# matteobutano/optimal_crowds

Hardware: NVIDIA B200
Metric: hjb_gcell_updates_per_s (higher is better)
Workload: dtype f64

## Files before the change

### include/optimal_crowds.h

```cpp
#ifndef OPTIMAL_CROWDS_H
#define OPTIMAL_CROWDS_H

#include <stdint.h>

#ifdef __cplusplus
extern "C" {
#endif

#define OC_ABI_VERSION 2

typedef enum {
    OC_OK = 0,
    OC_ERR_CUDA = -1,
    OC_ERR_ARG = -2,
    OC_ERR_NOMEM = -3,
    OC_ERR_SAMPLER_RANGE = -4,
    OC_ERR_STEP_TOO_SMALL = -5,
    OC_ERR_NCCL = -6
} oc_status;

typedef struct oc_ctx oc_ctx;

int oc_abi_version(void);
const char *oc_last_error(void);
long long oc_launch_count(int reset);

int oc_ctx_create(int device, int Ny, int Nx, double dx, double dy, double room_length, double room_height,
                  const double *X, const double *Y, oc_ctx **out);
void oc_ctx_destroy(oc_ctx *ctx);
int oc_ctx_set_int(oc_ctx *ctx, const char *key, int value);

int oc_upload(oc_ctx *ctx, const void *host, void *d_dst, long long bytes, void *stream);

long long oc_place_box(const double *box, const double *X, int Nx, const double *Y, int Ny, double *place_ped, double r_in,
                       uint32_t *mt_key, int *mt_pos, double *xs, double *ys, int loc_N);

int oc_rng_step_draw(uint32_t *mt_key, int *mt_pos, int *has_gauss, double *cached_gauss, int N, int n_active, int *perm,
                     double *noise);
int oc_rng_step_draw_ckpt(uint32_t *mt_key, int *mt_pos, int *has_gauss, double *cached_gauss, int N, int n_active,
                          int *perm, double *noise, int n_ckpt, uint32_t *ckpt_key, int *ckpt_pos, int *ckpt_has,
                          double *ckpt_cached);

int oc_rasterise(oc_ctx *ctx, const double *walls, int n_walls, const double *holes, int n_holes,
                 const double *cyls, int n_cyls, const double *targets, int n_targets, int remap,
                 double wall_value, double target_value, double *d_V, void *stream);

typedef struct {
    double sigma, mu, g;
    double rtol, atol;
    double lim;
    int fused;
    int profile;
    const double *forced_h;
    int n_forced_h;
    int chunk_rows;
} oc_hjb_params;

typedef struct {
    int nfev;
    int n_accepted;
    int n_rejected;
    int status;
    int n_out;
    int launches;
    double h0;
    double gpu_ms;
    int cls_launches[3];
    int pad_;
    double cls_ms[3];
    double cls_bytes[3];
} oc_hjb_stats;

int oc_hjb_solve(oc_ctx *ctx, const double *d_V, const double *d_m, const oc_hjb_params *prm, double T,
                 const double *t_eval, int nt, double *d_phi, double *d_vx, double *d_vy, oc_hjb_stats *stats,
                 double *trace_h, double *trace_err, int trace_cap, int *trace_n, void *stream);

int oc_hjb_plan_chunk_rows(oc_ctx *ctx, int copies);
int oc_hjb_solve_batch(oc_ctx *ctx, int n_rooms, const double *const *d_V, const double *const *d_m,
                       const oc_hjb_params *prm, double T, const double *t_eval, int nt, double *const *d_phi,
                       double *const *d_vx, double *const *d_vy, oc_hjb_stats *stats, void *stream);

typedef struct {
    int n_virtual;
    int own0, own1;
    int phi_extra_hi;
} oc_band_cfg;
int oc_dist_unique_id(void *out128);
int oc_dist_init(oc_ctx *ctx, const void *id128, int rank, int nranks);
int oc_dist_finalize(oc_ctx *ctx);
int oc_dist_p2p_export(oc_ctx *ctx, int band_rows, void *handle_out64);
int oc_dist_p2p_import(oc_ctx *ctx, const void *handles, int n);
int oc_dist_p2p_enabled(oc_ctx *ctx);
int oc_dist_p2p_disable(oc_ctx *ctx);
int oc_hjb_solve_band(oc_ctx *ctx, const oc_band_cfg *cfg, const double *d_V, const double *d_m,
                      const oc_hjb_params *prm, double T, const double *t_eval, int nt, double *d_phi, double *d_vx,
                      double *d_vy, oc_hjb_stats *stats, double *trace_h, double *trace_err, int trace_cap,
                      int *trace_n, void *stream);
int oc_rasterise_band(oc_ctx *ctx, const double *walls, int n_walls, const double *holes, int n_holes,
                      const double *cyls, int n_cyls, const double *targets, int n_targets, int remap,
                      double wall_value, double target_value, int row0, int rows, double *d_V, void *stream);

int oc_hjb_rhs(oc_ctx *ctx, const double *d_phi, const double *d_V, const double *d_m, const oc_hjb_params *prm,
               double *d_out, void *stream);
int oc_hjb_vels(oc_ctx *ctx, const double *d_phi, const oc_hjb_params *prm, double *d_vx, double *d_vy,
                void *stream);

typedef struct {
    double dt, dt2, half_noise, relaxation, v_max, cutoff;
    double a_min, tau_a, b_min, b_max, eta, eta_walls;
    double cos_fov, one_minus_cos_fov;
    double dx, dy, room_length, room_height;
    int Ny, Nx;
    int own0, own1;
    int key_mod, key_rem;
} oc_gcfm_params;

typedef struct {
    const double *d_V;
    const uint8_t *d_wall_tiles;
    double v_min;
    const double *d_vx, *d_vy;
    int nt_opt;
    int n_slices;
    const double *d_phi;
    int n_phi;
    int pad_;
    double mu, lim;
    const double *doors;
// ... 54 lines not shown
```

### optimal_crowds_b200/_lib.py

```python
from __future__ import annotations

import ctypes as C
import os

import numpy as np

_HERE = os.path.dirname(os.path.abspath(__file__))
LIB_PATH = os.environ.get("OC_B200_LIB") or os.path.join(_HERE, "liboc_b200.so")

dp = C.POINTER(C.c_double)
ip = C.POINTER(C.c_int)
u8p = C.POINTER(C.c_uint8)


class OcError(RuntimeError):
    def __init__(self, code, msg):
        super().__init__(f"liboc_b200 error {code}: {msg}")
        self.code = code


OC_ERR_SAMPLER_RANGE = -4
OC_ERR_STEP_TOO_SMALL = -5


class HjbParams(C.Structure):
    _fields_ = [("sigma", C.c_double), ("mu", C.c_double), ("g", C.c_double), ("rtol", C.c_double),
                ("atol", C.c_double), ("lim", C.c_double), ("fused", C.c_int), ("profile", C.c_int),
                ("forced_h", dp), ("n_forced_h", C.c_int), ("chunk_rows", C.c_int)]

    def force_steps(self, h):
        if h is None:
            self._keep = None
            self.forced_h, self.n_forced_h = None, 0
        else:
            self._keep = np.ascontiguousarray(h, dtype=np.float64)
            self.forced_h, self.n_forced_h = self._keep.ctypes.data_as(dp), len(self._keep)
        return self


class HjbStats(C.Structure):
    _fields_ = [("nfev", C.c_int), ("n_accepted", C.c_int), ("n_rejected", C.c_int), ("status", C.c_int),
                ("n_out", C.c_int), ("launches", C.c_int), ("h0", C.c_double), ("gpu_ms", C.c_double),
                ("cls_launches", C.c_int * 3), ("pad_", C.c_int), ("cls_ms", C.c_double * 3),
                ("cls_bytes", C.c_double * 3)]

    def asdict(self):
        d = {f: getattr(self, f) for f, _ in self._fields_ if not f.startswith(("cls_", "pad_"))}
        for f in ("cls_launches", "cls_ms", "cls_bytes"):
            d[f] = list(getattr(self, f))
        return d


class BandCfg(C.Structure):
    _fields_ = [("n_virtual", C.c_int), ("own0", C.c_int), ("own1", C.c_int), ("phi_extra_hi", C.c_int)]


class GcfmParams(C.Structure):
    _fields_ = [(n, C.c_double) for n in
                ("dt", "dt2", "half_noise", "relaxation", "v_max", "cutoff", "a_min", "tau_a", "b_min", "b_max",
                 "eta", "eta_walls", "cos_fov", "one_minus_cos_fov", "dx", "dy", "room_length", "room_height")] + \
               [("Ny", C.c_int), ("Nx", C.c_int), ("own0", C.c_int), ("own1", C.c_int), ("key_mod", C.c_int),
                ("key_rem", C.c_int)]


class Key(C.Structure):
    _fields_ = [("d_V", C.c_void_p), ("d_wall_tiles", C.c_void_p), ("v_min", C.c_double), ("d_vx", C.c_void_p),
                ("d_vy", C.c_void_p), ("nt_opt", C.c_int), ("n_slices", C.c_int), ("d_phi", C.c_void_p),
                ("n_phi", C.c_int), ("pad_", C.c_int), ("mu", C.c_double), ("lim", C.c_double), ("doors", dp),
                ("n_doors", C.c_int), ("phi_row0", C.c_int), ("phi_rows", C.c_int)]


_lib = None

EXPORTS = ["oc_abi_version", "oc_last_error", "oc_launch_count", "oc_ctx_create", "oc_ctx_destroy", "oc_ctx_set_int", "oc_rasterise",
           "oc_hjb_solve", "oc_hjb_rhs", "oc_hjb_vels", "oc_wall_tiles_bytes", "oc_wall_tiles", "oc_gcfm_step",
           "oc_wall_force", "oc_pair_force", "oc_density", "oc_gcfm_last_ms", "oc_dist_unique_id", "oc_dist_init",
           "oc_dist_finalize", "oc_dist_p2p_export", "oc_dist_p2p_import", "oc_dist_p2p_enabled", "oc_dist_p2p_disable", "oc_hjb_solve_band", "oc_rasterise_band", "oc_upload", "oc_hjb_solve_batch", "oc_gcfm_step_launch",
           "oc_gcfm_step_finish", "oc_gcfm_last_pairs", "oc_gcfm_last_redos", "oc_state_pack", "oc_fp64_peak", "oc_place_box", "oc_hjb_plan_chunk_rows", "oc_rng_step_draw", "oc_rng_step_draw_ckpt", "oc_gcfm_step_multi_launch", "oc_gcfm_step_multi_finish", "oc_gcfm_run"]


def load():
    global _lib
    if _lib is not None:
        return _lib
    if not os.path.exists(LIB_PATH):
        raise ImportError(f"{LIB_PATH} not found: build it with `python -m optimal_crowds_b200.build` "
                          "(the CUDA library is the only implementation; there is no CPU fallback)")
    lib = C.CDLL(LIB_PATH)
    lib.oc_last_error.restype = C.c_char_p
    lib.oc_launch_count.restype = C.c_longlong
    lib.oc_wall_tiles_bytes.restype = C.c_longlong
    lib.oc_gcfm_last_ms.restype = C.c_double
    lib.oc_gcfm_last_ms.argtypes = [C.c_void_p]
    lib.oc_gcfm_last_pairs.restype = C.c_longlong
    lib.oc_gcfm_last_pairs.argtypes = [C.c_void_p]
    lib.oc_gcfm_last_redos.argtypes = [C.c_void_p]
    lib.oc_state_pack.argtypes = [C.c_void_p, C.c_int] + [C.c_void_p] * 6
    lib.oc_fp64_peak.argtypes = [C.c_void_p, dp]
    lib.oc_hjb_plan_chunk_rows.argtypes = [C.c_void_p, C.c_int]
    vpp_ = C.POINTER(C.c_void_p)
    lib.oc_gcfm_step_multi_launch.argtypes = [C.c_int, vpp_, vpp_, ip] + [vpp_] * 9 + [ip, vpp_, ip, ip, dp, ip, ip,
                                                                                     C.c_int, C.c_void_p]
    lib.oc_gcfm_step_multi_finish.argtypes = [C.c_int, vpp_, vpp_, ip, ip]
    lib.oc_gcfm_run.argtypes = [C.c_void_p, C.POINTER(GcfmParams), C.c_int] + [C.c_void_p] * 8 + [C.c_void_p, C.c_int,
                                C.POINTER(C.c_uint32), ip, ip, dp, C.c_int, C.c_int, C.c_int, vpp_, ip, ip, ip, ip, dp,
                                C.POINTER(C.c_longlong), C.c_void_p]
    lib.oc_rng_step_draw.argtypes = [C.POINTER(C.c_uint32), ip, ip, dp, C.c_int, C.c_int, ip, dp]
    lib.oc_rng_step_draw_ckpt.argtypes = [C.POINTER(C.c_uint32), ip, ip, dp, C.c_int, C.c_int, ip, dp, C.c_int,
                                          C.POINTER(C.c_uint32), ip, ip, dp]
    lib.oc_place_box.restype = C.c_longlong
    lib.oc_place_box.argtypes = [dp, dp, C.c_int, dp, C.c_int, dp, C.c_double, C.POINTER(C.c_uint32), ip, dp, dp, C.c_int]
    lib.oc_wall_tiles_bytes.argtypes = [C.c_void_p]
    lib.oc_ctx_set_int.argtypes = [C.c_void_p, C.c_char_p, C.c_int]
    lib.oc_ctx_destroy.restype = None
    lib.oc_ctx_destroy.argtypes = [C.c_void_p]
    lib.oc_ctx_create.argtypes = [C.c_int, C.c_int, C.c_int, C.c_double, C.c_double, C.c_double, C.c_double, dp, dp,
                                  C.POINTER(C.c_void_p)]
    lib.oc_rasterise.argtypes = [C.c_void_p, dp, C.c_int, dp, C.c_int, dp, C.c_int, dp, C.c_int, C.c_int, C.c_double,
                                 C.c_double, C.c_void_p, C.c_void_p]
    lib.oc_hjb_solve.argtypes = [C.c_void_p, C.c_void_p, C.c_void_p, C.POINTER(HjbParams), C.c_double, dp, C.c_int,
                                 C.c_void_p, C.c_void_p, C.c_void_p, C.POINTER(HjbStats), dp, dp, C.c_int, ip,
                                 C.c_void_p]
    lib.oc_hjb_solve_band.argtypes = [C.c_void_p, C.POINTER(BandCfg), C.c_void_p, C.c_void_p, C.POINTER(HjbParams),
                                      C.c_double, dp, C.c_int, C.c_void_p, C.c_void_p, C.c_void_p, C.POINTER(HjbStats),
                                      dp, dp, C.c_int, ip, C.c_void_p]
    lib.oc_rasterise_band.argtypes = [C.c_void_p, dp, C.c_int, dp, C.c_int, dp, C.c_int, dp, C.c_int, C.c_int,
                                      C.c_double, C.c_double, C.c_int, C.c_int, C.c_void_p, C.c_void_p]
    vpp = C.POINTER(C.c_void_p)
    lib.oc_hjb_solve_batch.argtypes = [C.c_void_p, C.c_int, vpp, vpp, C.POINTER(HjbParams), C.c_double, dp, C.c_int,
                                       vpp, vpp, vpp, C.POINTER(HjbStats), C.c_void_p]
    lib.oc_upload.argtypes = [C.c_void_p, C.c_void_p, C.c_void_p, C.c_longlong, C.c_void_p]
    lib.oc_dist_unique_id.argtypes = [C.c_void_p]
    lib.oc_dist_init.argtypes = [C.c_void_p, C.c_void_p, C.c_int, C.c_int]
    lib.oc_dist_finalize.argtypes = [C.c_void_p]
    lib.oc_dist_p2p_export.argtypes = [C.c_void_p, C.c_int, C.c_void_p]
    lib.oc_dist_p2p_import.argtypes = [C.c_void_p, C.c_void_p, C.c_int]
    lib.oc_dist_p2p_enabled.argtypes = [C.c_void_p]
    lib.oc_dist_p2p_disable.argtypes = [C.c_void_p]
    lib.oc_hjb_rhs.argtypes = [C.c_void_p, C.c_void_p, C.c_void_p, C.c_void_p, C.POINTER(HjbParams), C.c_void_p,
                               C.c_void_p]
    lib.oc_hjb_vels.argtypes = [C.c_void_p, C.c_void_p, C.POINTER(HjbParams), C.c_void_p, C.c_void_p, C.c_void_p]
    lib.oc_wall_tiles.argtypes = [C.c_void_p, C.c_void_p, C.c_void_p, dp, C.c_void_p]
    lib.oc_gcfm_step.argtypes = [C.c_void_p, C.POINTER(GcfmParams), C.c_int] + [C.c_void_p] * 8 + \
                                [C.POINTER(Key), C.c_int, ip, dp, C.c_int, C.c_int, ip, ip, C.c_void_p]
    lib.oc_gcfm_step_launch.argtypes = [C.c_void_p, C.POINTER(GcfmParams), C.c_int] + [C.c_void_p] * 8 + \
                                       [C.POINTER(Key), C.c_int, ip, dp, C.c_int, C.c_int, C.c_void_p]
    lib.oc_gcfm_step_finish.argtypes = [C.c_void_p, ip, ip]
    lib.oc_wall_force.argtypes = [C.c_void_p, C.POINTER(GcfmParams), C.c_void_p, C.c_int] + [C.c_void_p] * 8 + \
                                 [C.c_void_p]
    lib.oc_pair_force.argtypes = [C.c_void_p, C.POINTER(GcfmParams), C.c_int] + [C.c_void_p] * 6 + [C.c_void_p]
    lib.oc_density.argtypes = [C.c_void_p, C.c_int, C.c_void_p, C.c_void_p, C.c_void_p, C.c_double, C.c_double,
                               C.c_void_p, C.c_void_p, C.c_void_p]
    _lib = lib
    return lib


def check(rc, allow=()):
    if rc != 0 and rc not in allow:
        raise OcError(rc, load().oc_last_error().decode())
    return rc


def _hp(a):
    return None if a is None else a.ctypes.data_as(dp)


def _dev(t):
    if t is None:
        return None
    assert t.is_cuda and t.is_contiguous(), "expected a contiguous CUDA tensor"
    return C.c_void_p(t.data_ptr())


def _stream():
    import torch
# ... 100 lines not shown
        t_eval = np.linspace(T, 0, nt)
        if n_virtual and n_virtual > 1 or own is None:
            rows, prow, own0, own1 = self.Ny, self.Ny, 0, self.Ny
            vshape = (max(nt - 1, 0), self.Ny - 2, self.Nx - 2)
        else:
            own0, own1 = own
            rows = own1 - own0
            prow = rows + 2 + int(phi_extra_hi)
            vshape = (max(nt - 1, 0), rows, self.Nx - 2)
        phi = out_phi if out_phi is not None else (self.empty(nt, prow, self.Nx) if want_phi else None)
        vx = vy = None
        if want_vel:
            import torch
            vx = torch.zeros(vshape, dtype=torch.float64, device=self.torch_device)
            vy = torch.zeros(vshape, dtype=torch.float64, device=self.torch_device)
        cfg = BandCfg(int(n_virtual or 0), int(own0), int(own1), int(phi_extra_hi))
        st = HjbStats()
        cap = 1 << 16 if trace else 0
        th = np.empty(max(cap, 1)); te = np.empty(max(cap, 1))
        ntr = C.c_int()
        rc = load().oc_hjb_solve_band(self.h, C.byref(cfg), _dev(V), _dev(m), C.byref(prm), float(T), _hp(t_eval),
                                      int(nt), _dev(phi), _dev(vx), _dev(vy), C.byref(st), _hp(th) if trace else None,
                                      _hp(te) if trace else None, cap, C.byref(ntr), _stream())
        check(rc, allow=(OC_ERR_STEP_TOO_SMALL,))
        res = {"stats": st.asdict(), "phi": phi, "vx": vx, "vy": vy, "rc": rc}
        if trace:
            k = min(ntr.value, cap)
            res["trace_h"], res["trace_err"] = th[:k].copy(), te[:k].copy()
        return res

    def hjb_solve(self, V, m, prm: HjbParams, T, nt, want_phi=False, want_vel=True, trace=False, out_vx=None,
                  out_vy=None, out_phi=None):
        t_eval = np.linspace(T, 0, nt)
        n = self.Ny * self.Nx
        phi = out_phi if out_phi is not None else (self.empty(nt, self.Ny, self.Nx) if want_phi else None)
        vx = vy = None
        if want_vel:
            vx = out_vx if out_vx is not None else self.empty(max(nt - 1, 0), self.Ny - 2, self.Nx - 2)
            vy = out_vy if out_vy is not None else self.empty(max(nt - 1, 0), self.Ny - 2, self.Nx - 2)
        st = HjbStats()
        cap = 1 << 16 if trace else 0
        th = np.empty(max(cap, 1)); te = np.empty(max(cap, 1))
        ntr = C.c_int()
        rc = load().oc_hjb_solve(self.h, _dev(V), _dev(m), C.byref(prm), float(T), _hp(t_eval), int(nt), _dev(phi),
                                 _dev(vx), _dev(vy), C.byref(st), _hp(th) if trace else None,
                                 _hp(te) if trace else None, cap, C.byref(ntr), _stream())
        check(rc, allow=(OC_ERR_STEP_TOO_SMALL,))
        res = {"stats": st.asdict(), "phi": phi, "vx": vx, "vy": vy, "rc": rc}
        if trace:
            k = min(ntr.value, cap)
            res["trace_h"], res["trace_err"] = th[:k].copy(), te[:k].copy()
        return res

    def hjb_solve_batch(self, Vs, ms, prm: HjbParams, T, nt, out_phi=None, out_vx=None, out_vy=None, want_vel=False):
        B = len(Vs)
        t_eval = np.linspace(T, 0, nt)
        if out_phi is None and not (want_vel or out_vx is not None):
            out_phi = [self.empty(nt, self.Ny, self.Nx) for _ in range(B)]
        if want_vel and out_vx is None:
            out_vx = [self.empty(max(nt - 1, 0), self.Ny - 2, self.Nx - 2) for _ in range(B)]
            out_vy = [self.empty(max(nt - 1, 0), self.Ny - 2, self.Nx - 2) for _ in range(B)]

        def ptrs(ts):
            if ts is None:
                return None
            arr = (C.c_void_p * B)()
            for q, t in enumerate(ts):
                if t is not None:
                    assert t.is_cuda and t.is_contiguous()
                    arr[q] = t.data_ptr()
            return arr
        st = (HjbStats * B)()
        rc = load().oc_hjb_solve_batch(self.h, B, ptrs(Vs), ptrs(ms), C.byref(prm), float(T), _hp(t_eval), int(nt),
                                       ptrs(out_phi), ptrs(out_vx), ptrs(out_vy), st, _stream())
        check(rc, allow=(OC_ERR_STEP_TOO_SMALL,))
        return [{"stats": st[q].asdict(), "phi": out_phi[q] if out_phi is not None else None,
                 "vx": out_vx[q] if out_vx is not None else None, "vy": out_vy[q] if out_vx is not None else None,
                 "rc": rc if st[q].status == -1 else 0} for q in range(B)]

    def plan_chunk_rows(self, copies=1):
        rc = int(load().oc_hjb_plan_chunk_rows(self.h, int(copies)))
        check(min(rc, 0))
        return rc

    def hjb_rhs(self, phi, V, m, prm: HjbParams):
        out = self.empty(self.Ny, self.Nx)
        check(load().oc_hjb_rhs(self.h, _dev(phi), _dev(V), _dev(m), C.byref(prm), _dev(out), _stream()))
        return out

    def hjb_vels(self, phi, prm: HjbParams):
        vx = self.empty(self.Ny - 2, self.Nx - 2); vy = self.empty(self.Ny - 2, self.Nx - 2)
        check(load().oc_hjb_vels(self.h, _dev(phi), C.byref(prm), _dev(vx), _dev(vy), _stream()))
        return vx, vy

    def wall_tiles(self, V):
        import torch
        nb = load().oc_wall_tiles_bytes(self.h)
        tiles = torch.empty(nb, dtype=torch.uint8, device=self.torch_device)
        vmin = C.c_double()
        check(load().oc_wall_tiles(self.h, _dev(V), _dev(tiles), C.byref(vmin), _stream()))
        return tiles, vmin.value

    def gcfm_step(self, prm: GcfmParams, state, vdes, key_id, keys, perm, noise, simu_step):
        return self.gcfm_step_finish(self.gcfm_step_launch(prm, state, vdes, key_id, keys, perm, noise, simu_step))

    @staticmethod
# ... 202 lines not shown
```

### optimal_crowds_b200/csrc/oc_hjb.cu

```cuda
#include <cmath>
#include <algorithm>
#include <vector>

#include "oc_common.h"
#include "oc_hjb_fused.cuh"
#include "oc_hjb_final.h"
#include "oc_rk45.h"
#include "oc_vels.h"

namespace {

constexpr int TX = 128, TY = 16, NTHREADS = 256;
constexpr int SW = TX + 2;

struct Comb {
    const double *y;
    const double *k[6];
    double a[6];
    double h;
};

template <int N>
__device__ __forceinline__ double comb_eval(const Comb &c, size_t idx) {
    if (N == 0) return c.y[idx];
    double acc = 0.0;
#pragma unroll
    for (int j = 0; j < N; j++) acc += __ldg(c.k[j] + idx) * c.a[j];
    return c.y[idx] + acc * c.h;
}

struct ErrArgs {
    const double *k[6];
    double e[7];
    double h, rtol, atol;
};

__device__ __forceinline__ double block_sum(double v, double *red) {
#pragma unroll
    for (int o = 16; o > 0; o >>= 1) v += __shfl_down_sync(0xffffffffu, v, o);
    int w = threadIdx.x >> 5, l = threadIdx.x & 31;
    if (l == 0) red[w] = v;
    __syncthreads();
    double s = 0.0;
    if (threadIdx.x == 0) {
#pragma unroll
        for (int i = 0; i < NTHREADS / 32; i++) s += red[i];
    }
    return s;
}

template <int N, int MODE>
__global__ void __launch_bounds__(NTHREADS)
hjb_stage_kernel(Comb c, const double *__restrict__ coef, double *__restrict__ kout, double *__restrict__ ynew,
                 ErrArgs ea, double *__restrict__ partial, int Ny, int Nx, double diff_over_dxdy) {
    __shared__ double tile[(TY + 2) * SW];
    __shared__ double red[NTHREADS / 32];
    const int tx0 = blockIdx.x * TX, ty0 = blockIdx.y * TY;
    for (int idx = threadIdx.x; idx < (TY + 2) * SW; idx += NTHREADS) {
        int ly = idx / SW, lx = idx - ly * SW;
        int gy = ty0 + ly - 1, gx = tx0 + lx - 1;
        if (gy < 0) gy = 1;
        if (gy == Ny) gy = Ny - 2;
        if (gx < 0) gx = 1;
        if (gx == Nx) gx = Nx - 2;
        double v = 0.0;
        if (gy < Ny && gx < Nx) v = comb_eval<N>(c, (size_t)gy * Nx + gx);
        tile[idx] = v;
    }
    __syncthreads();
    double acc = 0.0;
    const int lx = threadIdx.x & (TX - 1);
    const int gx = tx0 + lx;
#pragma unroll 2
    for (int ly = threadIdx.x / TX; ly < TY; ly += NTHREADS / TX) {
        int gy = ty0 + ly;
        if (gy >= Ny || gx >= Nx) continue;
        size_t g = (size_t)gy * Nx + gx;
        const double *t = tile + (ly + 1) * SW + (lx + 1);
        double C = t[0];
        double lap = t[-SW] + t[SW] + t[-1] + t[1] - 4.0 * C;
        double cf = coef[g];
        double r = diff_over_dxdy * lap - cf * C;
        if (cf != cf) r = 0.0;
        kout[g] = r;
        if (MODE == 1) {
            ynew[g] = C;
            double e = r * ea.e[6];
#pragma unroll
            for (int j = 5; j >= 0; j--)
                if (j != 1) e += __ldg(ea.k[j] + g) * ea.e[j];
            double sc = ea.atol + fmax(fabs(c.y[g]), fabs(C)) * ea.rtol;
            double q = (e * ea.h) / sc;
            acc += q * q;
        }
    }
    if (MODE == 1) {
        double s = block_sum(acc, red);
        if (threadIdx.x == 0) partial[(size_t)blockIdx.y * gridDim.x + blockIdx.x] = s;
    }
}

__global__ void __launch_bounds__(NTHREADS) rowgroup_sum_kernel(const double *__restrict__ partial, int nbx,
                                                                double *__restrict__ rowsum) {
    __shared__ double red[NTHREADS / 32];
    double v = 0.0;
    for (int i = threadIdx.x; i < nbx; i += NTHREADS) v += partial[(size_t)blockIdx.x * nbx + i];
    double s = block_sum(v, red);
    if (threadIdx.x == 0) rowsum[blockIdx.x] = s;
}

__global__ void __launch_bounds__(NTHREADS)
init_norm_kernel(const double *__restrict__ y, const double *__restrict__ f0, const double *__restrict__ f1,
                 double rtol, double atol, int Ny, int Nx, double *__restrict__ partial, int mode) {
    __shared__ double red[NTHREADS / 32];
    const int tx0 = blockIdx.x * TX, ty0 = blockIdx.y * TY;
    const int gx = tx0 + (threadIdx.x & (TX - 1));
    double a0 = 0.0, a1 = 0.0;
    for (int ly = threadIdx.x / TX; ly < TY; ly += NTHREADS / TX) {
        int gy = ty0 + ly;
        if (gy >= Ny || gx >= Nx) continue;
        size_t g = (size_t)gy * Nx + gx;
        double sc = atol + fabs(y[g]) * rtol;
        if (mode == 0) {
            double q0 = y[g] / sc, q1 = f0[g] / sc;
            a0 += q0 * q0;
            a1 += q1 * q1;
        } else {
            double q = (f1[g] - f0[g]) / sc;
            a0 += q * q;
        }
    }
    size_t nb = (size_t)gridDim.x * gridDim.y, b = (size_t)blockIdx.y * gridDim.x + blockIdx.x;
    double s0 = block_sum(a0, red);
    if (threadIdx.x == 0) partial[b] = s0;
    __syncthreads();
    if (mode == 0) {
        double s1 = block_sum(a1, red);
        if (threadIdx.x == 0) partial[nb + b] = s1;
    }
}

__global__ void prep_kernel(const double *__restrict__ V, const double *__restrict__ m, double g, double inv_den,
                            size_t n, double *__restrict__ coef, double *__restrict__ y) {
    size_t i = (size_t)blockIdx.x * blockDim.x + threadIdx.x;
    if (i >= n) return;
    double v = V[i];
    double mm = m ? m[i] : 0.0;
    coef[i] = (v < 0) ? __longlong_as_double(0x7ff8000000000000LL) : (v + g * mm) * inv_den;
    if (y) y[i] = 1.0;
}

constexpr int DTX = 64, DTY = 8, DSW = DTX + 2, DMAX = 6;
constexpr int DCELLS = (DTY + 2) * DSW;
constexpr int DPER = (DCELLS + NTHREADS - 1) / NTHREADS;

struct DenseArgs {
    const double *yold;
    const double *k[7];
    double P[7][4];
    double h;
    int n_emit;
    double x[DMAX];
    double *phi[DMAX];
    double *vx[DMAX];
    double *vy[DMAX];
    double mu, lim, inv_two_dx, inv_two_dy;
};

__global__ void __launch_bounds__(NTHREADS) hjb_dense_kernel(DenseArgs a, int Ny, int Nx) {
    __shared__ double tile[DCELLS];
    const int tx0 = blockIdx.x * DTX, ty0 = blockIdx.y * DTY;
    double q[DPER][4], y0[DPER];
#pragma unroll
    for (int s = 0; s < DPER; s++) {
        int idx = threadIdx.x + s * NTHREADS;
        q[s][0] = q[s][1] = q[s][2] = q[s][3] = 0.0;
        y0[s] = 0.0;
        if (idx < DCELLS) {
            int ly = idx / DSW, lx = idx - ly * DSW;
            int gy = ty0 + ly - 1, gx = tx0 + lx - 1;
            if (gy >= 0 && gy < Ny && gx >= 0 && gx < Nx) {
                size_t g = (size_t)gy * Nx + gx;
                y0[s] = a.yold[g];
#pragma unroll
                for (int j = 0; j < 7; j++) {
                    if (j == 1) continue;
                    double kj = __ldg(a.k[j] + g);
#pragma unroll
                    for (int p = 0; p < 4; p++) q[s][p] += kj * a.P[j][p];
                }
            }
        }
    }
    for (int e = 0; e < a.n_emit; e++) {
        double x = a.x[e];
        double p1 = x, p2 = p1 * x, p3 = p2 * x, p4 = p3 * x;
        __syncthreads();
#pragma unroll
        for (int s = 0; s < DPER; s++) {
            int idx = threadIdx.x + s * NTHREADS;
            if (idx < DCELLS) {
                double d = q[s][0] * p1 + q[s][1] * p2 + q[s][2] * p3 + q[s][3] * p4;
// ... 94 lines not shown
            case 1: launch_stage<1, 0>(c, kout, nullptr, ea); break;
            case 2: launch_stage<2, 0>(c, kout, nullptr, ea); break;
            case 3: launch_stage<3, 0>(c, kout, nullptr, ea); break;
            case 4: launch_stage<4, 0>(c, kout, nullptr, ea); break;
            case 5: launch_stage<5, 0>(c, kout, nullptr, ea); break;
        }
    }
    int fused_rc = 0, fused_gx = 0, fused_gy = 0;
    void fused_plan(int n_sm, int forced_rc = 0) {
        fused_gx = (Nx + fused::VX - 1) / fused::VX;
        fused_rc = forced_rc > 0 ? forced_rc : fused::plan_chunk_rows(Nx, Ny, n_sm, 1, 0);
        fused_gy = (Ny + fused_rc - 1) / fused_rc;
    }
    fused::MapCache maps;
    int launch_fused(int ne, fused::Args &a) {
        fused::set_tensor_maps(a, Ny, &maps);
        dim3 grid(fused_gx, fused_gy);
        begin(0, 8.0 * (double)n * (5 + ne));
        OC_CUDA(fused::launch<false>(ne, a, grid, st));
        end();
        launches++;
        return OC_OK;
    }
    int reduce_to_host(size_t off, double *out, int gx = -1, int gy = -1) {
        if (gx < 0) { gx = nbx; gy = nby; }
        begin(2, 8.0 * ((double)gx * gy + gy));
        rowgroup_sum_kernel<<<gy, NTHREADS, 0, st>>>(partial + off, gx, rowsum_d);
        end();
        launches++;
        OC_CUDA(cudaMemcpyAsync(rowsum_h, rowsum_d, sizeof(double) * gy, cudaMemcpyDeviceToHost, st));
        OC_CUDA(cudaStreamSynchronize(st));
        double s = 0.0;
        for (int i = 0; i < gy; i++) s += rowsum_h[i];
        *out = s;
        return OC_OK;
    }
};

int ensure_ws(oc_ctx *ctx, size_t n, int nbx, int nby) {
    int rc = oc_ensure_buffer(ctx->hjb_ws, ctx->hjb_ws_bytes, 10 * n * sizeof(double), false, "HJB workspace");
    if (rc) return rc;
    size_t np = (size_t)2 * nbx * nby + nby + 64;
    {
        size_t fgx = (size_t)(nbx * TX + fused::VX - 1) / fused::VX + 1, fgy = (size_t)(nby * TY + 15) / 16 + 1;
        np = std::max(np, 2 * fgx * fgy + fgy + 64);
    }
    if ((rc = oc_ensure_buffer(ctx->hjb_partial, ctx->hjb_partial_bytes, np * sizeof(double), false, "HJB partial sums")))
        return rc;
    size_t hp = (size_t)std::max(nby, (nby * TY + 15) / 16 + 1) + 16;
    return oc_ensure_buffer(ctx->h_pinned, ctx->h_pinned_bytes, hp * sizeof(double), true, "pinned host scratch");
}

int ensure_final_reduce(oc_ctx *ctx, int slots) { return ocfinal::ensure(ctx, slots); }
void final_reduce_args(oc_ctx *ctx, int slot, fused::Args &fa) { ocfinal::set_args(ctx, slot, ++ctx->fr_seq, fa); }
inline bool final_ready(oc_ctx *ctx, int slot, unsigned long long seq, double *out) { return ocfinal::ready(ctx, slot, seq, out); }
int wait_final(oc_ctx *ctx, int slot, unsigned long long seq, cudaStream_t st, double *out) {
    return ocfinal::wait(ctx, slot, seq, st, out);
}

}

extern "C" int oc_hjb_rhs(oc_ctx *ctx, const double *d_phi, const double *d_V, const double *d_m,
                          const oc_hjb_params *prm, double *d_out, void *stream) {
    OC_ARG(ctx && d_phi && d_V && prm && d_out, "NULL argument");
    OC_CUDA(cudaSetDevice(ctx->device));
    Solver s{};
    s.ctx = ctx; s.st = (cudaStream_t)stream; s.Ny = ctx->Ny; s.Nx = ctx->Nx;
    s.n = (size_t)s.Ny * s.Nx;
    s.nbx = (s.Nx + TX - 1) / TX; s.nby = (s.Ny + TY - 1) / TY;
    int rc = ensure_ws(ctx, s.n, s.nbx, s.nby);
    if (rc) return rc;
    s.coef = ctx->hjb_ws;
    s.partial = ctx->hjb_partial;
    double s2 = prm->sigma * prm->sigma;
    s.diff_over_dxdy = (-0.5 * s2) / (ctx->dx * ctx->dy);
    prep_kernel<<<(unsigned)((s.n + 255) / 256), 256, 0, s.st>>>(d_V, d_m, prm->g, 1.0 / (prm->mu * s2), s.n, s.coef, nullptr);
    Comb c{};
    c.y = d_phi;
    s.stage(0, c, d_out);
    oc::count_launch(2);
    OC_CUDA(cudaGetLastError());
    return OC_OK;
}

extern "C" int oc_hjb_plan_chunk_rows(oc_ctx *ctx, int copies) {
    if (!ctx || copies < 1) return OC_ERR_ARG;
    int n_sm = 148;
    cudaDeviceGetAttribute(&n_sm, cudaDevAttrMultiProcessorCount, ctx->device);
    return fused::plan_chunk_rows(ctx->Nx, ctx->Ny, n_sm, copies, 0);
}

extern "C" int oc_hjb_vels(oc_ctx *ctx, const double *d_phi, const oc_hjb_params *prm, double *d_vx, double *d_vy,
                           void *stream) {
    OC_ARG(ctx && d_phi && prm && d_vx && d_vy, "NULL argument");
    OC_CUDA(cudaSetDevice(ctx->device));
    dim3 grid((ctx->Nx - 2 + 63) / 64, (ctx->Ny - 2 + 3) / 4);
    vels_kernel<<<grid, NTHREADS, 0, (cudaStream_t)stream>>>(d_phi, ctx->Ny, ctx->Nx, prm->mu, prm->lim,
                                                             1.0 / (2 * ctx->dx), 1.0 / (2 * ctx->dy), d_vx, d_vy);
    oc::count_launch();
    OC_CUDA(cudaGetLastError());
    return OC_OK;
}

extern "C" int oc_hjb_solve(oc_ctx *ctx, const double *d_V, const double *d_m, const oc_hjb_params *prm, double T,
                            const double *t_eval, int nt, double *d_phi, double *d_vx, double *d_vy,
                            oc_hjb_stats *stats, double *trace_h, double *trace_err, int trace_cap, int *trace_n,
                            void *stream) {
    OC_ARG(ctx && d_V && prm && stats, "NULL argument");
    OC_ARG(nt >= 1 && t_eval, "t_eval required");
    OC_CUDA(cudaSetDevice(ctx->device));
    Solver s{};
    s.ctx = ctx; s.st = (cudaStream_t)stream; s.Ny = ctx->Ny; s.Nx = ctx->Nx;
    const size_t n = s.n = (size_t)s.Ny * s.Nx;
    s.nbx = (s.Nx + TX - 1) / TX; s.nby = (s.Ny + TY - 1) / TY;
    int rc = ensure_ws(ctx, n, s.nbx, s.nby);
    if (rc) return rc;
    double *ws = ctx->hjb_ws;
    s.coef = ws; s.y = ws + n; s.ynew = ws + 2 * n;
    for (int j = 0; j < 7; j++) s.K[j] = ws + (3 + j) * n;
    s.partial = ctx->hjb_partial;
    s.rowsum_d = ctx->hjb_partial + (size_t)2 * s.nbx * s.nby;
    s.rowsum_h = ctx->h_pinned;
    const double s2 = prm->sigma * prm->sigma;
    s.diff_over_dxdy = (-0.5 * s2) / (ctx->dx * ctx->dy);
    const double rtol = prm->rtol, atol = prm->atol;
    const double sqrt_n = std::sqrt((double)n);
    memset(stats, 0, sizeof(*stats));
    s.profile = prm->profile != 0;
    OC_CUDA(cudaEventRecord(ctx->ev0, s.st));

    prep_kernel<<<(unsigned)((n + 255) / 256), 256, 0, s.st>>>(d_V, d_m, prm->g, 1.0 / (prm->mu * s2), n, s.coef, s.y);
    s.launches++;
    rk45::Controller ctl(T, t_eval, nt);
    {
        Comb c{};
        c.y = s.y;
        s.stage(0, c, s.K[0]);
        stats->nfev++;
    }
    if (ctl.needs_initial_step()) {
        dim3 grid(s.nbx, s.nby);
        init_norm_kernel<<<grid, NTHREADS, 0, s.st>>>(s.y, s.K[0], nullptr, rtol, atol, s.Ny, s.Nx, s.partial, 0);
        s.launches++;
        double s0, s1, sq2;
        if ((rc = s.reduce_to_host(0, &s0))) return rc;
        if ((rc = s.reduce_to_host((size_t)s.nbx * s.nby, &s1))) return rc;
        const double d1 = std::sqrt(s1) / sqrt_n;
        const double h0 = ctl.initial_h0(std::sqrt(s0) / sqrt_n, d1);
        Comb c{};
        c.y = s.y; c.k[0] = s.K[0]; c.a[0] = 1.0; c.h = h0 * ctl.direction;
        s.stage(1, c, s.K[1]);
        stats->nfev++;
        init_norm_kernel<<<grid, NTHREADS, 0, s.st>>>(s.y, s.K[0], s.K[1], rtol, atol, s.Ny, s.Nx, s.partial, 1);
        s.launches++;
        if ((rc = s.reduce_to_host(0, &sq2))) return rc;
        ctl.set_initial_step(h0, d1, std::sqrt(sq2) / sqrt_n / h0);
    }
    stats->h0 = ctl.h_abs;

    bool use_fused = prm->fused != 0 && s.Ny > fused::HY + 1 && s.Nx > fused::HX + 1, fused_attempt = false;
    double *phi_scratch = nullptr;
    if (use_fused) {
        int n_sm = 148;
        cudaDeviceGetAttribute(&n_sm, cudaDevAttrMultiProcessorCount, ctx->device);
        s.fused_plan(n_sm, prm->chunk_rows);
        size_t np_need = (size_t)2 * s.fused_gx * s.fused_gy + s.fused_gy;
        if (ctx->hjb_partial_bytes < np_need * sizeof(double) || ctx->h_pinned_bytes < ((size_t)s.fused_gy + 16) * sizeof(double)) {
            oc::set_error("internal: fused partial buffers too small");
            return OC_ERR_ARG;
        }
        if (!d_phi && d_vx && d_vy) {
            size_t need = (size_t)fused::NE_MAX * n * sizeof(double);
            if ((rc = oc_ensure_buffer(ctx->hjb_scratch, ctx->hjb_scratch_bytes, need, false, "phi scratch"))) return rc;
            phi_scratch = ctx->hjb_scratch;
        }
    }
    const size_t n_int = (size_t)(s.Ny - 2) * (s.Nx - 2);
    const bool final_in_kernel = use_fused && s.fused_gy <= fused::MAX_FINAL_ROWS;
    if (final_in_kernel && (rc = ensure_final_reduce(ctx, 1))) return rc;
    const bool want_out = d_phi || (d_vx && d_vy);

    while (ctl.begin_step()) {
        bool accepted = false;
        while (!accepted && ctl.propose(prm->forced_h, prm->n_forced_h)) {
            const double h = ctl.h;
            fused_attempt = use_fused && (!want_out || d_phi || ctl.n_emit() <= fused::NE_MAX);
            double se;
            if (fused_attempt) {
                fused::Args fa{};
                fa.y = s.y; fa.k1 = s.K[0]; fa.coef = s.coef; fa.ynew = s.ynew; fa.k7 = s.K[6]; fa.partial = s.partial;
                fa.A = s.diff_over_dxdy; fa.rtol = rtol; fa.atol = atol;
                fa.Ny = s.Ny; fa.Nx = s.Nx; fa.RC = s.fused_rc;
                fa.row_base = 0; fa.own0 = 0; fa.own1 = s.Ny; fa.phi_row_base = 0;
                const int n_emit = want_out ? ctl.n_emit() : 0;
                int e0 = 0;
                do {
                    const int ne = std::min(n_emit - e0, fused::NE_MAX);
                    fused::set_attempt(fa, ctl, e0, ne, d_phi, phi_scratch, n);
                    if (final_in_kernel) final_reduce_args(ctx, 0, fa);
                    if ((rc = s.launch_fused(ne, fa))) return rc;
                    e0 += ne;
                } while (e0 < n_emit);
                stats->nfev += 6;
                if (final_in_kernel) {
                    if ((rc = wait_final(ctx, 0, fa.seq, s.st, &se))) return rc;
                } else if ((rc = s.reduce_to_host(0, &se, s.fused_gx, s.fused_gy))) return rc;
            } else {
            for (int sgi = 1; sgi < 6; sgi++) {
                Comb c{};
                c.y = s.y; c.h = h;
// ... 390 lines not shown
```

Baseline: 458.6.

## Fuse HJB solver prologue into two init kernels with on-device final reduction

Replaces the prologue sequence (prep kernel, stage-0 RHS, norm kernel, two host reductions, stage-1 RHS, norm kernel, host reduction) with two fused kernels. The first computes the coefficients, the initial state and the first RHS together with its norms. The second computes the trial-step RHS and the difference norm. Each kernel ends with a last-block ticket reduction that writes totals to mapped host memory, so fewer launches, memory passes and round-trip reductions are needed. The old path stays available behind a stagewise_prologue flag, and a standalone oc_hjb_initial_step entry point is added. The prologue is a small part of a full solve, so any change to end-to-end throughput may be small.

```diff
diff --git a/include/optimal_crowds.h b/include/optimal_crowds.h
--- a/include/optimal_crowds.h
+++ b/include/optimal_crowds.h
@@ -54,6 +54,7 @@
     const double *forced_h;
     int n_forced_h;
     int chunk_rows;
+    int stagewise_prologue;
 } oc_hjb_params;
 
 typedef struct {
@@ -74,6 +75,9 @@
 int oc_hjb_solve(oc_ctx *ctx, const double *d_V, const double *d_m, const oc_hjb_params *prm, double T,
                  const double *t_eval, int nt, double *d_phi, double *d_vx, double *d_vy, oc_hjb_stats *stats,
                  double *trace_h, double *trace_err, int trace_cap, int *trace_n, void *stream);
+
+int oc_hjb_initial_step(oc_ctx *ctx, const double *d_V, const double *d_m, const oc_hjb_params *prm, double T,
+                        double *d_coef, double *d_f0, double *out, void *stream);
 
 int oc_hjb_plan_chunk_rows(oc_ctx *ctx, int copies);
 int oc_hjb_solve_batch(oc_ctx *ctx, int n_rooms, const double *const *d_V, const double *const *d_m,
diff --git a/optimal_crowds_b200/_lib.py b/optimal_crowds_b200/_lib.py
--- a/optimal_crowds_b200/_lib.py
+++ b/optimal_crowds_b200/_lib.py
@@ -26,7 +26,7 @@
 class HjbParams(C.Structure):
     _fields_ = [("sigma", C.c_double), ("mu", C.c_double), ("g", C.c_double), ("rtol", C.c_double),
                 ("atol", C.c_double), ("lim", C.c_double), ("fused", C.c_int), ("profile", C.c_int),
-                ("forced_h", dp), ("n_forced_h", C.c_int), ("chunk_rows", C.c_int)]
+                ("forced_h", dp), ("n_forced_h", C.c_int), ("chunk_rows", C.c_int), ("stagewise_prologue", C.c_int)]
 
     def force_steps(self, h):
         if h is None:
@@ -76,7 +76,8 @@
            "oc_hjb_solve", "oc_hjb_rhs", "oc_hjb_vels", "oc_wall_tiles_bytes", "oc_wall_tiles", "oc_gcfm_step",
            "oc_wall_force", "oc_pair_force", "oc_density", "oc_gcfm_last_ms", "oc_dist_unique_id", "oc_dist_init",
            "oc_dist_finalize", "oc_dist_p2p_export", "oc_dist_p2p_import", "oc_dist_p2p_enabled", "oc_dist_p2p_disable", "oc_hjb_solve_band", "oc_rasterise_band", "oc_upload", "oc_hjb_solve_batch", "oc_gcfm_step_launch",
-           "oc_gcfm_step_finish", "oc_gcfm_last_pairs", "oc_gcfm_last_redos", "oc_state_pack", "oc_fp64_peak", "oc_place_box", "oc_hjb_plan_chunk_rows", "oc_rng_step_draw", "oc_rng_step_draw_ckpt", "oc_gcfm_step_multi_launch", "oc_gcfm_step_multi_finish", "oc_gcfm_run"]
+           "oc_gcfm_step_finish", "oc_gcfm_last_pairs", "oc_gcfm_last_redos", "oc_state_pack", "oc_fp64_peak", "oc_place_box", "oc_hjb_plan_chunk_rows", "oc_rng_step_draw", "oc_rng_step_draw_ckpt", "oc_gcfm_step_multi_launch", "oc_gcfm_step_multi_finish", "oc_gcfm_run",
+           "oc_hjb_initial_step"]
 
 
 def load():
@@ -121,6 +122,8 @@
     lib.oc_hjb_solve.argtypes = [C.c_void_p, C.c_void_p, C.c_void_p, C.POINTER(HjbParams), C.c_double, dp, C.c_int,
                                  C.c_void_p, C.c_void_p, C.c_void_p, C.POINTER(HjbStats), dp, dp, C.c_int, ip,
                                  C.c_void_p]
+    lib.oc_hjb_initial_step.argtypes = [C.c_void_p, C.c_void_p, C.c_void_p, C.POINTER(HjbParams), C.c_double,
+                                        C.c_void_p, C.c_void_p, dp, C.c_void_p]
     lib.oc_hjb_solve_band.argtypes = [C.c_void_p, C.POINTER(BandCfg), C.c_void_p, C.c_void_p, C.POINTER(HjbParams),
                                       C.c_double, dp, C.c_int, C.c_void_p, C.c_void_p, C.c_void_p, C.POINTER(HjbStats),
                                       dp, dp, C.c_int, ip, C.c_void_p]
@@ -327,6 +330,13 @@
             res["trace_h"], res["trace_err"] = th[:k].copy(), te[:k].copy()
         return res
 
+    def hjb_initial_step(self, V, m, prm: HjbParams, T):
+        coef, f0 = self.empty(self.Ny, self.Nx), self.empty(self.Ny, self.Nx)
+        out = np.zeros(4)
+        check(load().oc_hjb_initial_step(self.h, _dev(V), _dev(m), C.byref(prm), float(T), _dev(coef), _dev(f0),
+                                         _hp(out), _stream()))
+        return {"coef": coef, "f0": f0, "sums": out[:3].copy(), "h_abs": float(out[3])}
+
     def hjb_solve_batch(self, Vs, ms, prm: HjbParams, T, nt, out_phi=None, out_vx=None, out_vy=None, want_vel=False):
         B = len(Vs)
         t_eval = np.linspace(T, 0, nt)
diff --git a/optimal_crowds_b200/csrc/oc_hjb.cu b/optimal_crowds_b200/csrc/oc_hjb.cu
--- a/optimal_crowds_b200/csrc/oc_hjb.cu
+++ b/optimal_crowds_b200/csrc/oc_hjb.cu
@@ -48,6 +48,18 @@
     }
     return s;
 }
+
+__device__ __forceinline__ double stage_rhs(const double *t, double cf, double diff_over_dxdy) {
+    double C = t[0];
+    double lap = t[-SW] + t[SW] + t[-1] + t[1] - 4.0 * C;
+    double r = diff_over_dxdy * lap - cf * C;
+    if (cf != cf) r = 0.0;
+    return r;
+}
+__device__ __forceinline__ double coef_of(double v, double mm, double g, double inv_den) {
+    return (v < 0) ? __longlong_as_double(0x7ff8000000000000LL) : (v + g * mm) * inv_den;
+}
+__device__ __forceinline__ double init_scale(double y, double rtol, double atol) { return atol + fabs(y) * rtol; }
 
 template <int N, int MODE>
 __global__ void __launch_bounds__(NTHREADS)
@@ -78,10 +90,8 @@
         size_t g = (size_t)gy * Nx + gx;
         const double *t = tile + (ly + 1) * SW + (lx + 1);
         double C = t[0];
-        double lap = t[-SW] + t[SW] + t[-1] + t[1] - 4.0 * C;
         double cf = coef[g];
-        double r = diff_over_dxdy * lap - cf * C;
-        if (cf != cf) r = 0.0;
+        double r = stage_rhs(t, cf, diff_over_dxdy);
         kout[g] = r;
         if (MODE == 1) {
             ynew[g] = C;
@@ -120,7 +130,7 @@
         int gy = ty0 + ly;
         if (gy >= Ny || gx >= Nx) continue;
         size_t g = (size_t)gy * Nx + gx;
-        double sc = atol + fabs(y[g]) * rtol;
+        double sc = init_scale(y[g], rtol, atol);
         if (mode == 0) {
             double q0 = y[g] / sc, q1 = f0[g] / sc;
             a0 += q0 * q0;
@@ -144,10 +154,166 @@
                             size_t n, double *__restrict__ coef, double *__restrict__ y) {
     size_t i = (size_t)blockIdx.x * blockDim.x + threadIdx.x;
     if (i >= n) return;
-    double v = V[i];
-    double mm = m ? m[i] : 0.0;
-    coef[i] = (v < 0) ? __longlong_as_double(0x7ff8000000000000LL) : (v + g * mm) * inv_den;
+    coef[i] = coef_of(V[i], m ? m[i] : 0.0, g, inv_den);
     if (y) y[i] = 1.0;
+}
+
+struct InitArgs {
+    const double *V, *m;
+    double g, inv_den;
+    double *coef, *y, *f0;
+    double *f1;
+    double h;
+    double rtol, atol, diff_over_dxdy;
+    int Ny, Nx;
+    double *partial;
+    unsigned *ticket;
+    double *result[2];
+    unsigned long long seq;
+};
+
+template <int NSUM>
+__device__ void tile_partials_totals(const double *p, size_t stride, int gx, int gy, double *rows, double *tot) {
+    constexpr int RW = 2;
+    const int lane = threadIdx.x & 31, warp = threadIdx.x >> 5;
+    const int nv = NSUM * gy;
+#pragma unroll
+    for (int k = 0; k < NSUM; k++) tot[k] = 0.0;
+    for (int v0 = 0; v0 < nv; v0 += RW * NTHREADS / 32) {
+        double x[RW][8];
+        const double *src[RW];
+#pragma unroll
+        for (int q = 0; q < RW; q++) {
+            const int v = v0 + warp * RW + q, k = v / gy;
+            src[q] = p + k * stride + (size_t)(v - k * gy) * gx;
+#pragma unroll
+            for (int vw = 0; vw < 8; vw++) {
+                const int i = vw * 32 + lane;
+                x[q][vw] = (v < nv && i < gx) ? __ldcg(src[q] + i) : 0.0;
+            }
+        }
+#pragma unroll
+        for (int q = 0; q < RW; q++) {
+            const int v = v0 + warp * RW + q;
+            double srow = 0.0;
+#pragma unroll
+            for (int vw = 0; vw < 8; vw++) {
+                double acc = 0.0 + x[q][vw];
+                for (int i = vw * 32 + lane + NTHREADS; v < nv && i < gx; i += NTHREADS) acc += __ldcg(src[q] + i);
+#pragma unroll
+                for (int o = 16; o > 0; o >>= 1) acc += __shfl_down_sync(0xffffffffu, acc, o);
+                srow += acc;
+            }
+            if (lane == 0) rows[warp * RW + q] = srow;
+        }
+        __syncthreads();
+        if (threadIdx.x == 0)
+            for (int w = 0; w < RW * NTHREADS / 32 && v0 + w < nv; w++) tot[(v0 + w) / gy] += rows[w];
+        __syncthreads();
+    }
+}
+
+template <int PASS>
+__global__ void __launch_bounds__(NTHREADS, 3) hjb_init_kernel(InitArgs a) {
+    constexpr int RPT = TY / (NTHREADS / TX);
+    __shared__ double tile[(TY + 2) * SW];
+    __shared__ double red[2 * NTHREADS / 32];
+    __shared__ int is_last;
+    const int Ny = a.Ny, Nx = a.Nx;
+    const int tx0 = blockIdx.x * TX, ty0 = blockIdx.y * TY;
+    const int lx = threadIdx.x & (TX - 1), ly0 = threadIdx.x / TX;
+    const int gx = tx0 + lx;
+    bool in[RPT];
+    size_t gg[RPT];
+    double l0[RPT], l1[RPT], l2[RPT];
+#pragma unroll
+    for (int j = 0; j < RPT; j++) {
+        const int gy = ty0 + ly0 + 2 * j;
+        in[j] = gy < Ny && gx < Nx;
+        gg[j] = in[j] ? (size_t)gy * Nx + gx : 0;
+        if (PASS == 0) {
+            l0[j] = in[j] ? a.V[gg[j]] : 0.0;
+            l1[j] = (in[j] && a.m) ? a.m[gg[j]] : 0.0;
+            l2[j] = 0.0;
+        } else {
+            l0[j] = in[j] ? a.coef[gg[j]] : 0.0;
+            l1[j] = in[j] ? a.y[gg[j]] : 0.0;
+            l2[j] = in[j] ? a.f0[gg[j]] : 0.0;
+        }
+    }
+    Comb c{};
+    c.y = a.y; c.k[0] = a.f0; c.a[0] = 1.0; c.h = a.h;
+    constexpr int TILE = (TY + 2) * SW;
+#pragma unroll
+    for (int it = 0; it < (TILE + NTHREADS - 1) / NTHREADS; it++) {
+        const int idx = threadIdx.x + it * NTHREADS;
+        if (idx < TILE) {
+            int ly = idx / SW, lx2 = idx - ly * SW;
+            int gy = ty0 + ly - 1, gx2 = tx0 + lx2 - 1;
+            if (gy < 0) gy = 1;
+            if (gy == Ny) gy = Ny - 2;
+            if (gx2 < 0) gx2 = 1;
+            if (gx2 == Nx) gx2 = Nx - 2;
+            double v = 0.0;
+            if (gy < Ny && gx2 < Nx) v = PASS == 0 ? 1.0 : comb_eval<1>(c, (size_t)gy * Nx + gx2);
+            tile[idx] = v;
+        }
+    }
+    __syncthreads();
+    double a0 = 0.0, a1 = 0.0;
+#pragma unroll
+    for (int j = 0; j < RPT; j++) {
+        if (!in[j]) continue;
+        const size_t g = gg[j];
+        const double *t = tile + (ly0 + 2 * j + 1) * SW + (lx + 1);
+        double cf;
+        if (PASS == 0) {
+            cf = coef_of(l0[j], l1[j], a.g, a.inv_den);
+            a.coef[g] = cf;
+            a.y[g] = 1.0;
+        } else {
+            cf = l0[j];
+        }
+        const double r = stage_rhs(t, cf, a.diff_over_dxdy);
+        if (PASS == 0) {
+            a.f0[g] = r;
+            double sc = init_scale(1.0, a.rtol, a.atol);
+            double q0 = 1.0 / sc, q1 = r / sc;
+            a0 += q0 * q0;
+            a1 += q1 * q1;
+        } else {
+            if (a.f1) a.f1[g] = r;
+            double sc = init_scale(l1[j], a.rtol, a.atol);
+            double q = (r - l2[j]) / sc;
+            a0 += q * q;
+        }
+    }
+    const size_t nb = (size_t)gridDim.x * gridDim.y, b = (size_t)blockIdx.y * gridDim.x + blockIdx.x;
+    double s0 = block_sum(a0, red);
+    if (threadIdx.x == 0) a.partial[b] = s0;
+    __syncthreads();
+    if (PASS == 0) {
+        double s1 = block_sum(a1, red);
+        if (threadIdx.x == 0) a.partial[nb + b] = s1;
+    }
+    if (threadIdx.x == 0) {
+        __threadfence();
+        is_last = atomicAdd(a.ticket, 1u) == nb - 1;
+    }
+    __syncthreads();
+    if (!is_last) return;
+    __threadfence();
+    constexpr int NSUM = PASS == 0 ? 2 : 1;
+    double tot[NSUM];
+    tile_partials_totals<NSUM>(a.partial, nb, gridDim.x, gridDim.y, red, tot);
+    if (threadIdx.x == 0) {
+        *a.ticket = 0u;
+#pragma unroll
+        for (int k = 0; k < NSUM; k++) *reinterpret_cast<volatile double *>(a.result[k]) = tot[k];
+        __threadfence_system();
+#pragma unroll
+        for (int k = 0; k < NSUM; k++) *reinterpret_cast<volatile unsigned long long *>(a.result[k] + 1) = a.seq;
+    }
 }
 
 constexpr int DTX = 64, DTY = 8, DSW = DTX + 2, DMAX = 6;
@@ -348,10 +514,76 @@
 }
 
 int ensure_final_reduce(oc_ctx *ctx, int slots) { return ocfinal::ensure(ctx, slots); }
+
 void final_reduce_args(oc_ctx *ctx, int slot, fused::Args &fa) { ocfinal::set_args(ctx, slot, ++ctx->fr_seq, fa); }
 inline bool final_ready(oc_ctx *ctx, int slot, unsigned long long seq, double *out) { return ocfinal::ready(ctx, slot, seq, out); }
 int wait_final(oc_ctx *ctx, int slot, unsigned long long seq, cudaStream_t st, double *out) {
     return ocfinal::wait(ctx, slot, seq, st, out);
+}
+
+int prologue(Solver &s, rk45::Controller &ctl, const double *d_V, const double *d_m, const oc_hjb_params *prm,
+             oc_hjb_stats *stats, double *norms) {
+    oc_ctx *ctx = s.ctx;
+    const double s2 = prm->sigma * prm->sigma, rtol = prm->rtol, atol = prm->atol;
+    const double sqrt_n = std::sqrt((double)s.n);
+    double sum[3] = {0.0, 0.0, 0.0};
+    int rc;
+    const dim3 grid(s.nbx, s.nby);
+    if (prm->stagewise_prologue) {
+        prep_kernel<<<(unsigned)((s.n + 255) / 256), 256, 0, s.st>>>(d_V, d_m, prm->g, 1.0 / (prm->mu * s2), s.n, s.coef, s.y);
+        s.launches++;
+        Comb c{};
+        c.y = s.y;
+        s.stage(0, c, s.K[0]);
+        stats->nfev++;
+        if (ctl.needs_initial_step()) {
+            init_norm_kernel<<<grid, NTHREADS, 0, s.st>>>(s.y, s.K[0], nullptr, rtol, atol, s.Ny, s.Nx, s.partial, 0);
+            s.launches++;
+            if ((rc = s.reduce_to_host(0, &sum[0]))) return rc;
+            if ((rc = s.reduce_to_host((size_t)s.nbx * s.nby, &sum[1]))) return rc;
+            const double d1 = std::sqrt(sum[1]) / sqrt_n;
+            const double h0 = ctl.initial_h0(std::sqrt(sum[0]) / sqrt_n, d1);
+            c.k[0] = s.K[0]; c.a[0] = 1.0; c.h = h0 * ctl.direction;
+            s.stage(1, c, s.K[1]);
+            stats->nfev++;
+            init_norm_kernel<<<grid, NTHREADS, 0, s.st>>>(s.y, s.K[0], s.K[1], rtol, atol, s.Ny, s.Nx, s.partial, 1);
+            s.launches++;
+            if ((rc = s.reduce_to_host(0, &sum[2]))) return rc;
+            ctl.set_initial_step(h0, d1, std::sqrt(sum[2]) / sqrt_n / h0);
+        }
+    } else {
+        if ((rc = ensure_final_reduce(ctx, 2))) return rc;
+        double *res = nullptr;
+        OC_CUDA(cudaHostGetDevicePointer(&res, ctx->fr_result, 0));
+        InitArgs a{};
+        a.V = d_V; a.m = d_m; a.g = prm->g; a.inv_den = 1.0 / (prm->mu * s2);
+        a.coef = s.coef; a.y = s.y; a.f0 = s.K[0];
+        a.rtol = rtol; a.atol = atol; a.diff_over_dxdy = s.diff_over_dxdy;
+        a.Ny = s.Ny; a.Nx = s.Nx; a.partial = s.partial;
+        a.ticket = ctx->fr_ticket; a.result[0] = res; a.result[1] = res + 2;
+        a.seq = ++ctx->fr_seq;
+        s.begin(0, 8.0 * (double)s.n * (d_m ? 5 : 4));
+        hjb_init_kernel<0><<<grid, NTHREADS, 0, s.st>>>(a);
+        s.end();
+        s.launches++;
+        stats->nfev++;
+        if (ctl.needs_initial_step()) {
+            if ((rc = wait_final(ctx, 0, a.seq, s.st, &sum[0])) || (rc = wait_final(ctx, 1, a.seq, s.st, &sum[1]))) return rc;
+            const double d1 = std::sqrt(sum[1]) / sqrt_n;
+            const double h0 = ctl.initial_h0(std::sqrt(sum[0]) / sqrt_n, d1);
+            a.h = h0 * ctl.direction;
+            a.seq = ++ctx->fr_seq;
+            s.begin(0, 8.0 * (double)s.n * 3);
+            hjb_init_kernel<1><<<grid, NTHREADS, 0, s.st>>>(a);
+            s.end();
+            s.launches++;
+            stats->nfev++;
+            if ((rc = wait_final(ctx, 0, a.seq, s.st, &sum[2]))) return rc;
+            ctl.set_initial_step(h0, d1, std::sqrt(sum[2]) / sqrt_n / h0);
+        }
+    }
+    if (norms) for (int k = 0; k < 3; k++) norms[k] = sum[k];
+    return OC_OK;
 }
 
 }
@@ -375,6 +607,35 @@
     c.y = d_phi;
     s.stage(0, c, d_out);
     oc::count_launch(2);
+    OC_CUDA(cudaGetLastError());
+    return OC_OK;
+}
+
+extern "C" int oc_hjb_initial_step(oc_ctx *ctx, const double *d_V, const double *d_m, const oc_hjb_params *prm, double T,
+                                   double *d_coef, double *d_f0, double *out, void *stream) {
+    OC_ARG(ctx && d_V && prm && out, "NULL argument");
+    OC_CUDA(cudaSetDevice(ctx->device));
+    Solver s{};
+    s.ctx = ctx; s.st = (cudaStream_t)stream; s.Ny = ctx->Ny; s.Nx = ctx->Nx;
+    const size_t n = s.n = (size_t)s.Ny * s.Nx;
+    s.nbx = (s.Nx + TX - 1) / TX; s.nby = (s.Ny + TY - 1) / TY;
+    int rc = ensure_ws(ctx, n, s.nbx, s.nby);
+    if (rc) return rc;
+    double *ws = ctx->hjb_ws;
+    s.coef = ws; s.y = ws + n; s.ynew = ws + 2 * n;
+    for (int j = 0; j < 7; j++) s.K[j] = ws + (3 + j) * n;
+    s.partial = ctx->hjb_partial;
+    s.rowsum_d = ctx->hjb_partial + (size_t)2 * s.nbx * s.nby;
+    s.rowsum_h = ctx->h_pinned;
+    s.diff_over_dxdy = (-0.5 * prm->sigma * prm->sigma) / (ctx->dx * ctx->dy);
+    oc_hjb_stats stats{};
+    rk45::Controller ctl(T, nullptr, 0);
+    if ((rc = prologue(s, ctl, d_V, d_m, prm, &stats, out))) return rc;
+    out[3] = ctl.h_abs;
+    if (d_coef) OC_CUDA(cudaMemcpyAsync(d_coef, s.coef, n * sizeof(double), cudaMemcpyDeviceToDevice, s.st));
+    if (d_f0) OC_CUDA(cudaMemcpyAsync(d_f0, s.K[0], n * sizeof(double), cudaMemcpyDeviceToDevice, s.st));
+    OC_CUDA(cudaStreamSynchronize(s.st));
+    oc::count_launch(s.launches);
     OC_CUDA(cudaGetLastError());
     return OC_OK;
 }
@@ -425,33 +686,8 @@
     s.profile = prm->profile != 0;
     OC_CUDA(cudaEventRecord(ctx->ev0, s.st));
 
-    prep_kernel<<<(unsigned)((n + 255) / 256), 256, 0, s.st>>>(d_V, d_m, prm->g, 1.0 / (prm->mu * s2), n, s.coef, s.y);
-    s.launches++;
     rk45::Controller ctl(T, t_eval, nt);
-    {
-        Comb c{};
-        c.y = s.y;
-        s.stage(0, c, s.K[0]);
-        stats->nfev++;
-    }
-    if (ctl.needs_initial_step()) {
-        dim3 grid(s.nbx, s.nby);
-        init_norm_kernel<<<grid, NTHREADS, 0, s.st>>>(s.y, s.K[0], nullptr, rtol, atol, s.Ny, s.Nx, s.partial, 0);
-        s.launches++;
-        double s0, s1, sq2;
-        if ((rc = s.reduce_to_host(0, &s0))) return rc;
-        if ((rc = s.reduce_to_host((size_t)s.nbx * s.nby, &s1))) return rc;
-        const double d1 = std::sqrt(s1) / sqrt_n;
-        const double h0 = ctl.initial_h0(std::sqrt(s0) / sqrt_n, d1);
-        Comb c{};
-        c.y = s.y; c.k[0] = s.K[0]; c.a[0] = 1.0; c.h = h0 * ctl.direction;
-        s.stage(1, c, s.K[1]);
-        stats->nfev++;
-        init_norm_kernel<<<grid, NTHREADS, 0, s.st>>>(s.y, s.K[0], s.K[1], rtol, atol, s.Ny, s.Nx, s.partial, 1);
-        s.launches++;
-        if ((rc = s.reduce_to_host(0, &sq2))) return rc;
-        ctl.set_initial_step(h0, d1, std::sqrt(sq2) / sqrt_n / h0);
-    }
+    if ((rc = prologue(s, ctl, d_V, d_m, prm, stats, nullptr))) return rc;
     stats->h0 = ctl.h_abs;
 
     bool use_fused = prm->fused != 0 && s.Ny > fused::HY + 1 && s.Nx > fused::HX + 1, fused_attempt = false;
```

After: 466.4 (median of 6 runs). +1.7%, better.
